# verlab/accelerated_features

Hardware: AMD Instinct MI355X
Metric: frames/sec detectAndCompute+match (VGA, top_k=4096) (higher is better)
Workload: dtype f32; 1 GPU; VGA 640x480 sparse top_k=4096, batch=64 per GPU: detectAndCompute + MNN match of the 32 consecutive frame pairs (BASELINE configs[1]); batch_per_gpu=64, height=480, width=640, top_k=4096, weights=synthetic (tests/fixtures.py), barrier=none (one rank), concurrent_lanes=True, lanes=2

## Files before the change

### accelerated_features_amd/csrc/k_match_f16.hip

```cpp
#include "../../include/xfeat_hip.h"
#include "kernels.hpp"
#include <type_traits>

namespace xfh {

void prof_begin(Profiler* p, int which, hipStream_t st);
void prof_end(Profiler* p, int which, hipStream_t st, double flops, double bytes);

typedef float f32x16 __attribute__((ext_vector_type(16)));
typedef _Float16 f16x8 __attribute__((ext_vector_type(8)));
typedef _Float16 f16x4 __attribute__((ext_vector_type(4)));


constexpr int FT_COLS = 256;
constexpr int FT_DS = 72;
constexpr float F16_C = 1.03f * 0.0009765625f;
constexpr float F16_KAPPA = 1.0e-5f;
constexpr float F16_UNIT_SCALE = 256.f;

__device__ inline int fpair_count(const int32_t* n, int idx, int cap) {
    if (!n) return cap;
    const int v = n[idx];
    return v < 0 ? 0 : (v > cap ? cap : v);
}
__device__ inline float f16_scale(float maxnorm) {
    if (!(maxnorm > 0.f)) return 1.f;
    int e;
    (void)frexpf(maxnorm, &e);
    return ldexpf(1.f, 8 - e);
}

template <bool CVT>
__global__ __launch_bounds__(256) void mnn_prep_kernel(const float* __restrict__ d1, size_t ps1, const float* __restrict__ d2, size_t ps2,
                                                       const int32_t* __restrict__ n1p, const int32_t* __restrict__ n2p, int n_stride, int n_off2,
                                                       int N1, int N2, _Float16* __restrict__ a16, _Float16* __restrict__ b16,
                                                       float* __restrict__ na, float* __restrict__ nb, unsigned* __restrict__ nmax ) {
    __shared__ float wmax[4];
    const int p = blockIdx.y, side = blockIdx.z, P = gridDim.y;
    const int N = side ? N2 : N1;
    const int n = side ? fpair_count(n2p, p * n_stride + n_off2, N2) : fpair_count(n1p, p * n_stride, N1);
    const int sub = threadIdx.x & 15;
    if (blockIdx.x * 256 >= n) return;
    const float* src = (side ? d2 + (size_t)p * ps2 : d1 + (size_t)p * ps1);
    const float sc = CVT ? f16_scale(__uint_as_float(nmax[side * P + p])) : 0.f;
    float m = 0.f;
#pragma unroll 4
    for (int it = 0; it < 16; ++it) {
        const int row = blockIdx.x * 256 + it * 16 + (threadIdx.x >> 4);
        float s = 0.f;
        if (row < n) {
            const float4 v = *reinterpret_cast<const float4*>(src + (size_t)row * 64 + sub * 4);
            if (CVT) {
                f16x4 o;
                o[0] = (_Float16)(v.x * sc); o[1] = (_Float16)(v.y * sc); o[2] = (_Float16)(v.z * sc); o[3] = (_Float16)(v.w * sc);
                *reinterpret_cast<f16x4*>((side ? b16 : a16) + ((size_t)p * N + row) * 64 + sub * 4) = o;
            } else {
                s = v.x * v.x + v.y * v.y + v.z * v.z + v.w * v.w;
            }
        }
        if (!CVT) {
            s += __shfl_xor(s, 8, 64);
            s += __shfl_xor(s, 4, 64);
            s += __shfl_xor(s, 2, 64);
            s += __shfl_xor(s, 1, 64);
            const float nrm = sqrtf(s) * 1.000001f;
            if (row < n && sub == 0) (side ? nb : na)[(size_t)p * N + row] = nrm;
            if (row < n) m = fmaxf(m, nrm);
        }
    }
    if (!CVT) {
        m = fmaxf(m, __shfl_xor(m, 16, 64));
        m = fmaxf(m, __shfl_xor(m, 32, 64));
        if ((threadIdx.x & 63) == 0) wmax[threadIdx.x >> 6] = m;
        __syncthreads();
        if (threadIdx.x == 0)
            atomicMax(&nmax[side * P + p], __float_as_uint(fmaxf(fmaxf(wmax[0], wmax[1]), fmaxf(wmax[2], wmax[3]))));
    }
}

constexpr float F16_STORE_SCALE = 0.25f;
__device__ inline _Float16 f16_up(float x) { return (_Float16)(__builtin_fmaf(__builtin_fabsf(x), 0.0009765625f, x) + 5.9604644775390625e-8f); }
__device__ inline _Float16 f16_down(float x) { return (_Float16)(__builtin_fmaf(__builtin_fabsf(x), -0.0009765625f, x) - 5.9604644775390625e-8f); }

__device__ inline float max16(const f32x16& v) {
    const float a = fmaxf(fmaxf(v[0], v[1]), v[2]);
    const float b = fmaxf(fmaxf(v[3], v[4]), v[5]);
    const float c = fmaxf(fmaxf(v[6], v[7]), v[8]);
    const float d = fmaxf(fmaxf(v[9], v[10]), v[11]);
    const float e = fmaxf(fmaxf(v[12], v[13]), v[14]);
    const float f = fmaxf(fmaxf(a, b), c);
    const float g = fmaxf(fmaxf(d, e), v[15]);
    return fmaxf(f, g);
}

__device__ inline float xhalf_max(float v) {
    const auto r = __builtin_amdgcn_permlane32_swap(__float_as_uint(v), __float_as_uint(v), false, false);
    return fmaxf(__uint_as_float(r[0]), __uint_as_float(r[1]));
}

struct PairWindow { float two_c, two_k; };
__device__ inline PairWindow pair_window(float unit_bound, const unsigned* __restrict__ nmax, int P, int p, bool row_side) {
    PairWindow w;
    if (unit_bound > 0.f) {
        const float ss = F16_UNIT_SCALE * F16_UNIT_SCALE;
        w.two_c = 2.f * F16_C * ss * unit_bound;
        w.two_k = 2.f * F16_KAPPA * ss * unit_bound * unit_bound;
    } else {
        const float ma = __uint_as_float(nmax[p]), mb = __uint_as_float(nmax[P + p]);
        const float ss = f16_scale(ma) * f16_scale(mb);
        w.two_c = 2.f * F16_C * ss * (row_side ? mb : ma);
        w.two_k = 2.f * F16_KAPPA * ss * ma * mb;
    }
    w.two_c = __uint_as_float(__builtin_amdgcn_readfirstlane(__float_as_uint(w.two_c)));
    w.two_k = __uint_as_float(__builtin_amdgcn_readfirstlane(__float_as_uint(w.two_k)));
    return w;
}

#define XFH_KEEP_FRAGS(f) asm volatile("" :: "v"(f[0]), "v"(f[1]), "v"(f[2]), "v"(f[3]))
#define XFH_WAVE_SYNC() __builtin_amdgcn_wave_barrier()

constexpr int FT_TILES = FT_COLS / 32;
__global__ __launch_bounds__(512) void mnn_f16_sweep_kernel(const _Float16* __restrict__ a16, size_t sa16, const _Float16* __restrict__ b16, size_t sb16,
                                                            const int32_t* __restrict__ n1p, const int32_t* __restrict__ n2p, int n_stride, int n_off2,
                                                            int N1, int N2, int ncc, int nsplit, int P,
                                                            unsigned* __restrict__ colmaxh, unsigned* __restrict__ rowmaxh,
                                                            _Float16* __restrict__ R, _Float16* __restrict__ C
#if XFH_CODE_SHIFT > 0
                                                            , int cold
#endif
                                                            ) {
#if XFH_CODE_SHIFT > 0
    kernel_entry_hooks(cold);
#endif
    __shared__ __attribute__((aligned(16))) _Float16 Dl[FT_COLS * FT_DS];
    __shared__ float colx[8][FT_COLS];
    __shared__ int next_block;
    const int tid = threadIdx.x, lane = tid & 63, half = lane >> 5, l31 = lane & 31;
    const int wave = __builtin_amdgcn_readfirstlane(tid >> 6);
    int p, item;
    if (!xcd_group_map(blockIdx.x, ncc * nsplit, P, p, item)) return;
    const int cc = item / nsplit, rs = item - cc * nsplit;
    const int n1 = fpair_count(n1p, p * n_stride, N1);
    const int n2 = fpair_count(n2p, p * n_stride + n_off2, N2);
    const int c0 = cc * FT_COLS;
    if (n1 <= 0 || n2 <= 0 || c0 >= n2) return;
    const _Float16* A = a16 + (size_t)p * sa16;
    const _Float16* Bm = b16 + (size_t)p * sb16;
    const int ncb32 = ceil_div(N2, 32), nrb32 = ceil_div(N1, 32);
    const int ntile = min(FT_TILES, ceil_div(n2 - c0, 32));
    const int bps = ceil_div(ceil_div(n1, 32), nsplit);
    const int blk_lo = rs * bps, nblock = min(ceil_div(n1, 32), blk_lo + bps);
    if (blk_lo >= nblock) return;
    if (tid == 0) next_block = blk_lo + 8;
    {
        uint4 v[4];
#pragma unroll
        for (int i = 0; i < 4; ++i) {
            const int e = tid + i * 512;
            v[i] = *reinterpret_cast<const uint4*>(Bm + (size_t)min(c0 + (e >> 3), n2 - 1) * 64 + (e & 7) * 8);
        }
#pragma unroll
        for (int i = 0; i < 4; ++i) {
            const int e = tid + i * 512;
            *reinterpret_cast<uint4*>(Dl + (e >> 3) * FT_DS + (e & 7) * 8) = v[i];
        }
#pragma unroll
        for (int i = 0; i < 4; ++i) (&colx[0][0])[tid + i * 512] = -INFINITY;
    }
    f16x8 a[4], an[4];
    int blk = blk_lo + wave, nxt;
    if (blk < nblock) {
        const int row = min(blk * 32 + l31, n1 - 1);
#pragma unroll
        for (int kk = 0; kk < 4; ++kk) an[kk] = *reinterpret_cast<const f16x8*>(A + (size_t)row * 64 + kk * 16 + half * 8);
    }
    __syncthreads();
    float* mycolx = &colx[wave][l31];
    const _Float16* bp0 = Dl + l31 * FT_DS + half * 8;
    while (blk < nblock) {
        {
            int t = 0;
            if (lane == 0) t = atomicAdd(&next_block, 1);
            nxt = __builtin_amdgcn_readfirstlane(t);
        }
#pragma unroll
        for (int kk = 0; kk < 4; ++kk) a[kk] = an[kk];
        if (nxt < nblock) {
            const int row = min(nxt * 32 + l31, n1 - 1);
#pragma unroll
            for (int kk = 0; kk < 4; ++kk) an[kk] = *reinterpret_cast<const f16x8*>(A + (size_t)row * 64 + kk * 16 + half * 8);
        }
        const int myrow = blk * 32 + l31;
        const __amdgpu_buffer_rsrc_t rC = __builtin_amdgcn_make_buffer_rsrc(C + ((size_t)p * nrb32 + blk) * N2 + c0, 0, (min(n2, c0 + FT_COLS) - c0) * 2, 0x00020000);
        const __amdgpu_buffer_rsrc_t rR = __builtin_amdgcn_make_buffer_rsrc(R + ((size_t)p * ncb32 + (c0 >> 5)) * N1, 0, FT_TILES * N1 * 2, 0x00020000);
        const int offC = half == 0 ? l31 * 2 : (int)0x80000000;
        const int offR = (half == 1 && myrow < n1) ? myrow * 2 : (int)0x80000000;
        float rowrun = -INFINITY;
        f16x8 bfrag[2][4];
#pragma unroll
        for (int kk = 0; kk < 4; ++kk) bfrag[0][kk] = *reinterpret_cast<const f16x8*>(bp0 + kk * 16);
        f32x16 acc, accT;
#define XFH_ROW_EPILOGUE(CT)                                                                              \
        {                                                                                                 \
            float rm = max16(accT);                                                                       \
            rm = fmaxf(rm, xhalf(rm));                                                                    \
            rowrun = fmaxf(rowrun, rm);                                                                   \
            __builtin_amdgcn_raw_buffer_store_b16(__builtin_bit_cast(short, f16_up(rm * F16_STORE_SCALE)), rR, offR, (CT) * N1 * 2, 0);       \
        }
#define XFH_INTERLEAVE_4x5()                                                                              \
        __builtin_amdgcn_sched_group_barrier(0x008, 1, 0); __builtin_amdgcn_sched_group_barrier(0x002, 5, 0);   \
        __builtin_amdgcn_sched_group_barrier(0x008, 1, 0); __builtin_amdgcn_sched_group_barrier(0x002, 5, 0);   \
        __builtin_amdgcn_sched_group_barrier(0x008, 1, 0); __builtin_amdgcn_sched_group_barrier(0x002, 5, 0);   \
        __builtin_amdgcn_sched_group_barrier(0x008, 1, 0); __builtin_amdgcn_sched_group_barrier(0x002, 5, 0);
#pragma unroll
        for (int ct = 0; ct < FT_TILES; ++ct) {
            if (ct < ntile) {
                if (ct + 1 < FT_TILES) {
#pragma unroll
                    for (int kk = 0; kk < 4; ++kk) bfrag[(ct + 1) & 1][kk] = *reinterpret_cast<const f16x8*>(bp0 + (ct + 1) * 32 * FT_DS + kk * 16);
                }
#pragma unroll
                for (int r = 0; r < 16; ++r) acc[r] = 0.f;
#pragma unroll
                for (int kk = 0; kk < 4; ++kk) acc = __builtin_amdgcn_mfma_f32_32x32x16_f16(a[kk], bfrag[ct & 1][kk], acc, 0, 0, 0);
                if (ct > 0) XFH_ROW_EPILOGUE(ct - 1)
                XFH_INTERLEAVE_4x5()
                __builtin_amdgcn_sched_barrier(0);
#pragma unroll
                for (int r = 0; r < 16; ++r) accT[r] = 0.f;
#pragma unroll
                for (int kk = 0; kk < 4; ++kk) accT = __builtin_amdgcn_mfma_f32_32x32x16_f16(bfrag[ct & 1][kk], a[kk], accT, 0, 0, 0);
                {
                    float cm = max16(acc);
                    cm = fmaxf(cm, xhalf(cm));
                    __hip_atomic_fetch_max(mycolx + ct * 32, cm, __ATOMIC_RELAXED, __HIP_MEMORY_SCOPE_WORKGROUP);
                    __builtin_amdgcn_raw_buffer_store_b16(__builtin_bit_cast(short, f16_up(cm * F16_STORE_SCALE)), rC, offC + ct * 64, 0, 0);
                }
                XFH_INTERLEAVE_4x5()
                __builtin_amdgcn_sched_barrier(0);
                XFH_KEEP_FRAGS(bfrag[ct & 1]);
            }
        }
        XFH_ROW_EPILOGUE(ntile - 1)
#undef XFH_ROW_EPILOGUE
#undef XFH_INTERLEAVE_4x5
        if (half == 0 && myrow < n1) atomicMax(&rowmaxh[(size_t)p * N1 + myrow], float_ord(rowrun));
        blk = nxt;
    }
    __syncthreads();
    if (tid < FT_COLS && c0 + tid < n2) {
        float k = colx[0][tid];
#pragma unroll
        for (int w = 1; w < 8; ++w) k = fmaxf(k, colx[w][tid]);
        atomicMax(&colmaxh[(size_t)p * N2 + c0 + tid], float_ord(k));
    }
}

constexpr int S2_T = 32;
constexpr int S2_GROUP = 32 * S2_T;
constexpr int S2_WAVES = 4;
constexpr int S2_TILES = 4;
constexpr int S2_COLS = 32 * S2_TILES;
constexpr int S2_XP = 33;
__host__ __device__ inline int s2_c_blocks(int N1) { return ceil_div(N1, S2_GROUP) * 32; }
__global__ __launch_bounds__(64 * S2_WAVES) __attribute__((amdgpu_waves_per_eu(2, 2)))
void mnn_f16_sweep2_kernel(const _Float16* __restrict__ a16, size_t sa16, const _Float16* __restrict__ b16, size_t sb16,
                           const int32_t* __restrict__ n1p, const int32_t* __restrict__ n2p, int n_stride, int n_off2,
                           int N1, int N2, int ncc, int ngq, int P,
                           unsigned* __restrict__ colmaxh, unsigned* __restrict__ rowmaxh, _Float16* __restrict__ R, _Float16* __restrict__ C) {
    __shared__ __attribute__((aligned(16))) _Float16 Dl2[S2_COLS * FT_DS];
    __shared__ __attribute__((aligned(16))) _Float16 af[S2_WAVES][64 * FT_DS];
    const int tid = threadIdx.x, lane = tid & 63, half = lane >> 5, l31 = lane & 31;
    const int wave = __builtin_amdgcn_readfirstlane(tid >> 6);
    int p, item;
    if (!xcd_group_map(blockIdx.x, ncc * ngq, P, p, item)) return;
    const int cc = item / ngq, gq = item - cc * ngq;
    const int n1 = fpair_count(n1p, p * n_stride, N1);
    const int n2 = fpair_count(n2p, p * n_stride + n_off2, N2);
    const int c0 = cc * S2_COLS;
    if (n1 <= 0 || n2 <= 0 || c0 >= n2 || gq * S2_WAVES * S2_GROUP >= n1) return;
    const _Float16* A = a16 + (size_t)p * sa16;
    const _Float16* Bm = b16 + (size_t)p * sb16;
    const int ncb32 = ceil_div(N2, 32);
    {
        constexpr int NP = S2_COLS * 8 / (64 * S2_WAVES);
        uint4 v[NP];
#pragma unroll
        for (int i = 0; i < NP; ++i) {
            const int e = tid + i * (64 * S2_WAVES);
            v[i] = *reinterpret_cast<const uint4*>(Bm + (size_t)min(c0 + (e >> 3), n2 - 1) * 64 + (e & 7) * 8);
        }
#pragma unroll
        for (int i = 0; i < NP; ++i) {
            const int e = tid + i * (64 * S2_WAVES);
            *reinterpret_cast<uint4*>(Dl2 + (e >> 3) * FT_DS + (e & 7) * 8) = v[i];
        }
    }
    const int g = gq * S2_WAVES + wave;
    const int blk_lo = g * S2_T, nblock = min(ceil_div(n1, 32), blk_lo + S2_T);
    f16x8 ax[4], ay[4], anx[4], any_[4];
#define XFH_S2_REQUEST(BLK)                                                                                \
    {                                                                                                     \
         \
        _Pragma("unroll") for (int q = 0; q < 4; ++q) {                                                   \
            const int e = q * 64 + lane, rx = min((BLK) * 32 + (e >> 3), n1 - 1), ry = (BLK) + 1 < nblock ? min((BLK) * 32 + 32 + (e >> 3), n1 - 1) : rx;       \
            anx[q] = *reinterpret_cast<const f16x8*>(A + (size_t)rx * 64 + (e & 7) * 8);                  \
            any_[q] = *reinterpret_cast<const f16x8*>(A + (size_t)ry * 64 + (e & 7) * 8);                 \
        }                                                                                                 \
    }
    XFH_S2_REQUEST(min(blk_lo, max(nblock - 1, 0)))
    __syncthreads();
    if (blk_lo >= nblock) return;
    const _Float16* bp0 = Dl2 + l31 * FT_DS + half * 8;
    _Float16* afw = af[wave];
    f32x16 M[S2_TILES];
#pragma unroll
    for (int ct = 0; ct < S2_TILES; ++ct)
#pragma unroll
        for (int r = 0; r < 16; ++r) M[ct][r] = -INFINITY;
    const __amdgpu_buffer_rsrc_t rR = __builtin_amdgcn_make_buffer_rsrc(R + ((size_t)p * ncb32 + (c0 >> 5)) * N1, 0, min(S2_TILES, ncb32 - (c0 >> 5)) * N1 * 2, 0x00020000);
    constexpr int NSTEP = 4 * S2_TILES;
    f16x8 bq[4];
    bq[0] = *reinterpret_cast<const f16x8*>(bp0);
    bq[1] = *reinterpret_cast<const f16x8*>(bp0 + 16);
    for (int blk = blk_lo; blk < nblock; blk += 2) {
#pragma unroll
        for (int q = 0; q < 4; ++q) {
            const int e = q * 64 + lane;
            *reinterpret_cast<f16x8*>(afw + (e >> 3) * FT_DS + (e & 7) * 8) = anx[q];
            *reinterpret_cast<f16x8*>(afw + (32 + (e >> 3)) * FT_DS + (e & 7) * 8) = any_[q];
        }
        XFH_WAVE_SYNC();
#pragma unroll
        for (int kk = 0; kk < 4; ++kk) {
            ax[kk] = *reinterpret_cast<const f16x8*>(afw + l31 * FT_DS + kk * 16 + half * 8);
            ay[kk] = *reinterpret_cast<const f16x8*>(afw + (32 + l31) * FT_DS + kk * 16 + half * 8);
        }
        XFH_WAVE_SYNC();
        XFH_S2_REQUEST(min(blk + 2, nblock - 1))
        const int myrow = blk * 32 + lane;
        const int offR = myrow < n1 ? myrow * 2 : (int)0x80000000;
        const int arow = half && blk + 1 >= nblock ? min(blk * 32 + l31, n1 - 1) : min(myrow, n1 - 1);
        float rowrun = -INFINITY;
        f32x16 accx[2], accy[2];
#define XFH_S2_FENCE() __builtin_amdgcn_sched_barrier(0)
#define XFH_S2_M(CT, R0, R1) { _Pragma("unroll") for (int r = (R0); r < (R1); ++r) M[CT][r] = fmaxf(fmaxf(M[CT][r], accx[(CT) & 1][r]), accy[(CT) & 1][r]); }
#define XFH_S2_PIN2(CT, R0) asm volatile("" : "+v"(M[CT][R0]), "+v"(M[CT][(R0) + 1]))
#define XFH_S2_PIN10(CT, R0) asm volatile("" : "+v"(M[CT][R0]), "+v"(M[CT][(R0) + 1]), "+v"(M[CT][(R0) + 2]), "+v"(M[CT][(R0) + 3]), "+v"(M[CT][(R0) + 4]), "+v"(M[CT][(R0) + 5]), \
                                                "+v"(M[CT][(R0) + 6]), "+v"(M[CT][(R0) + 7]), "+v"(M[CT][(R0) + 8]), "+v"(M[CT][(R0) + 9]))
#define XFH_S2_EPI0(CT) rx_ = max16(accx[(CT) & 1]); XFH_S2_M(CT, 0, 2) XFH_S2_PIN2(CT, 0); asm volatile("" : "+v"(rx_));
#define XFH_S2_EPI1(CT) ry_ = max16(accy[(CT) & 1]); XFH_S2_M(CT, 2, 4) XFH_S2_PIN2(CT, 2); asm volatile("" : "+v"(ry_));
#define XFH_S2_EPI2(CT)                                                                                   \
            {                                                                                             \
                const auto sw_ = __builtin_amdgcn_permlane32_swap(__float_as_uint(rx_), __float_as_uint(ry_), false, false);       \
                const float rm_ = fmaxf(__uint_as_float(sw_[0]), __uint_as_float(sw_[1]));                \
                rowrun = fmaxf(rowrun, rm_);                                                              \
                __builtin_amdgcn_raw_buffer_store_b16(__builtin_bit_cast(short, f16_up(rm_ * F16_STORE_SCALE)), rR, offR + (CT) * N1 * 2, 0, 0);    \
            }                                                                                             \
            XFH_S2_M(CT, 4, 6) XFH_S2_PIN2(CT, 4); asm volatile("" : "+v"(rowrun));
#define XFH_S2_EPI3(CT) XFH_S2_M(CT, 6, 16) XFH_S2_PIN10(CT, 6);
        float rx_ = 0.f, ry_ = 0.f;
#pragma unroll
        for (int ct = 0; ct < S2_TILES; ++ct)
#pragma unroll
        for (int kk = 0; kk < 4; ++kk) {
            const int s_ = 4 * ct + kk;
            {
                const int sn = (s_ + 2) % NSTEP;
                bq[(s_ + 2) & 3] = *reinterpret_cast<const f16x8*>(bp0 + (sn >> 2) * 32 * FT_DS + (sn & 3) * 16);
            }
            f32x16& cx = accx[ct & 1];
            f32x16& cy = accy[ct & 1];
            if (kk == 0) {
#pragma unroll
                for (int r = 0; r < 16; ++r) { cx[r] = 0.f; cy[r] = 0.f; }
            }
            cx = __builtin_amdgcn_mfma_f32_32x32x16_f16(bq[s_ & 3], ax[kk], cx, 0, 0, 0);
            cy = __builtin_amdgcn_mfma_f32_32x32x16_f16(bq[s_ & 3], ay[kk], cy, 0, 0, 0);
            asm volatile("" : "+v"(cx), "+v"(cy));
            XFH_S2_FENCE();
            if (ct > 0) {
                if (kk == 0) { XFH_S2_EPI0(ct - 1) }
                if (kk == 1) { XFH_S2_EPI1(ct - 1) }
                if (kk == 2) { XFH_S2_EPI2(ct - 1) }
                if (kk == 3) { XFH_S2_EPI3(ct - 1) }
                XFH_S2_FENCE();
            }
            asm volatile("" :: "v"(bq[s_ & 3]));
        }
        {
            XFH_S2_EPI0(S2_TILES - 1)
            XFH_S2_EPI1(S2_TILES - 1)
            XFH_S2_EPI2(S2_TILES - 1)
            XFH_S2_EPI3(S2_TILES - 1)
        }
        XFH_S2_FENCE();
        XFH_KEEP_FRAGS(ax);
        XFH_KEEP_FRAGS(ay);
#undef XFH_S2_FENCE
#undef XFH_S2_PIN2
#undef XFH_S2_PIN10
#undef XFH_S2_M
#undef XFH_S2_EPI0
#undef XFH_S2_EPI1
#undef XFH_S2_EPI2
#undef XFH_S2_EPI3
        atomicMax(&rowmaxh[(size_t)p * N1 + arow], float_ord(rowrun));
    }
    float* xw = reinterpret_cast<float*>(af[wave]);
    static_assert(32 * S2_XP * 4 <= 64 * FT_DS * 2, "the flush tile lives in the wave's fragment rows");
    const bool vec_ok = (N2 & 7) == 0;
    _Float16* crow = C + ((size_t)p * s2_c_blocks(N1) + g * 32 + l31) * N2 + c0;
#pragma unroll
    for (int ct = 0; ct < S2_TILES; ++ct) {
#pragma unroll
        for (int r = 0; r < 16; ++r) xw[l31 * S2_XP + (r & 3) + 8 * (r >> 2) + 4 * half] = M[ct][r];
        XFH_WAVE_SYNC();
        float cm = xw[(16 * half) * S2_XP + l31];
#pragma unroll
        for (int t = 1; t < 16; ++t) cm = fmaxf(cm, xw[(16 * half + t) * S2_XP + l31]);
        cm = fmaxf(cm, xhalf(cm));
        const int col = c0 + ct * 32 + l31;
        if (half == 0 && col < n2) atomicMax(&colmaxh[(size_t)p * N2 + col], float_ord(cm));
        const int cs = ct * 32 + 16 * half;
        _Float16 o[16];
#pragma unroll
        for (int t = 0; t < 16; ++t) o[t] = f16_up(xw[l31 * S2_XP + 16 * half + t] * F16_STORE_SCALE);
#pragma unroll
        for (int q = 0; q < 2; ++q) {
            f16x8 v;
#pragma unroll
            for (int t = 0; t < 8; ++t) v[t] = o[8 * q + t];
            if (vec_ok && c0 + cs + 8 * q + 8 <= n2) *reinterpret_cast<f16x8*>(crow + cs + 8 * q) = v;
            else {
#pragma unroll
                for (int t = 0; t < 8; ++t)
                    if (c0 + cs + 8 * q + t < n2) crow[cs + 8 * q + t] = v[t];
            }
        }
        XFH_WAVE_SYNC();
    }
}

__global__ __launch_bounds__(256) void mnn_f16_thr_kernel(float unit_bound, const int32_t* __restrict__ n1p, const int32_t* __restrict__ n2p, int n_stride, int n_off2,
                                                          int N1, int N2, int P, const float* __restrict__ na, const float* __restrict__ nb,
                                                          const unsigned* __restrict__ nmax, const unsigned* __restrict__ rowmaxh, const unsigned* __restrict__ colmaxh,
                                                          _Float16* __restrict__ thr_row, _Float16* __restrict__ thr_col) {
    const int p = blockIdx.y, side = blockIdx.z, i = blockIdx.x * 256 + threadIdx.x;
    const int N = side ? N2 : N1;
    if (i >= (side ? fpair_count(n2p, p * n_stride + n_off2, N2) : fpair_count(n1p, p * n_stride, N1))) return;
    const PairWindow w = pair_window(unit_bound, nmax, P, p, side == 0);
    const float nx = unit_bound > 0.f ? unit_bound : (side ? nb : na)[(size_t)p * N + i];
    (side ? thr_col : thr_row)[(size_t)p * N + i] = f16_down((ord_float((side ? colmaxh : rowmaxh)[(size_t)p * N + i]) - fmaf(w.two_c, nx, w.two_k)) * F16_STORE_SCALE);
}

constexpr int RF_ROUND = 512;
constexpr int RF_CHUNK = 4096;
constexpr int RF_QUEUE = 1024;
constexpr int RF_XS = 68;
constexpr int RF_WAVES = 2;
__global__ __launch_bounds__(64 * RF_WAVES) __attribute__((amdgpu_waves_per_eu(4, 8))) void mnn_f16_refine_kernel(
    const float* __restrict__ d1, size_t ps1, const float* __restrict__ d2, size_t ps2, const int32_t* __restrict__ n1p,
    const int32_t* __restrict__ n2p, int n_stride, int n_off2, int N1, int N2, int nyb_max, int c_strided, int P,
    const _Float16* __restrict__ thr_row, const _Float16* __restrict__ thr_col, const _Float16* __restrict__ R,
    const _Float16* __restrict__ C, unsigned long long* __restrict__ rowkey, unsigned long long* __restrict__ colkey) {
    __shared__ unsigned short queue[RF_WAVES][RF_QUEUE];
    __shared__ __attribute__((aligned(16))) float tile[RF_WAVES][32 * RF_XS];
    const int lane = threadIdx.x & 63, half = lane >> 5, l31 = lane & 31;
    const int wv = __builtin_amdgcn_readfirstlane(threadIdx.x >> 6);
    int p, item;
    if (!xcd_group_map(blockIdx.x, 2 * (nyb_max / RF_WAVES), P, p, item)) return;
    const int side = item / (nyb_max / RF_WAVES), yb = (item - side * (nyb_max / RF_WAVES)) * RF_WAVES + wv;
    const int n1 = fpair_count(n1p, p * n_stride, N1);
    const int n2 = fpair_count(n2p, p * n_stride + n_off2, N2);
    if (n1 <= 0 || n2 <= 0) return;
    const int nX = side ? n2 : n1, nY = side ? n1 : n2, NX = side ? N2 : N1;
    const bool strided = side && c_strided;
    const int ybase = strided ? (yb >> 5) * S2_GROUP + (yb & 31) : yb * 32, ystep = strided ? 32 : 1;
    if (ybase >= nY) return;
    const float* X = side ? d2 + (size_t)p * ps2 : d1 + (size_t)p * ps1;
    const float* Y = side ? d1 + (size_t)p * ps1 : d2 + (size_t)p * ps2;
    const _Float16* M = (side ? C + (size_t)p * (c_strided ? s2_c_blocks(N1) : ceil_div(N1, 32)) * N2 : R + (size_t)p * ceil_div(N2, 32) * N1) + (size_t)yb * NX;
    const _Float16* T = side ? thr_col + (size_t)p * N2 : thr_row + (size_t)p * N1;
    unsigned long long* key = side ? colkey + (size_t)p * N2 : rowkey + (size_t)p * N1;
    const bool vec_ok = (NX & 7) == 0;
    unsigned short* q = queue[wv];
    float* xt = tile[wv];
    const __amdgpu_buffer_rsrc_t rM = __builtin_amdgcn_make_buffer_rsrc(const_cast<_Float16*>(M), 0, nX * 2, 0x00020000);
    const __amdgpu_buffer_rsrc_t rT = __builtin_amdgcn_make_buffer_rsrc(const_cast<_Float16*>(T), 0, nX * 2, 0x00020000);
    const __amdgpu_buffer_rsrc_t rX = __builtin_amdgcn_make_buffer_rsrc(const_cast<float*>(X), 0, nX * 256, 0x00020000);
    const __amdgpu_buffer_rsrc_t rY = __builtin_amdgcn_make_buffer_rsrc(const_cast<float*>(Y), 0, nY * 256, 0x00020000);

    const int trow = lane >> 4, tq = lane & 15;
    auto rows_to_operand = [&](const __amdgpu_buffer_rsrc_t& rs, auto row_of, float (&reg)[32]) {
        uint4 v[8];
#pragma unroll
        for (int i = 0; i < 8; ++i) v[i] = __builtin_bit_cast(uint4, __builtin_amdgcn_raw_buffer_load_b128(rs, row_of(4 * i + trow) * 256 + tq * 16, 0, 0));
#pragma unroll
        for (int i = 0; i < 8; ++i) *reinterpret_cast<uint4*>(xt + (4 * i + trow) * RF_XS + tq * 4) = v[i];
#pragma unroll
        for (int t = 0; t < 8; ++t) {
            const float4 f = *reinterpret_cast<const float4*>(xt + l31 * RF_XS + half * 32 + t * 4);
            reg[4 * t] = f.x; reg[4 * t + 1] = f.y; reg[4 * t + 2] = f.z; reg[4 * t + 3] = f.w;
        }
    };
    float yreg[32];
    rows_to_operand(rY, [&](int r) { return ybase + r * ystep; }, yreg);
    const bool ragged = ybase + 31 * ystep >= nY;

    for (int xc = 0; xc < nX; xc += RF_CHUNK) {
        int cnt = 0;
        auto drain = [&]() {
            for (int e0 = 0; e0 < cnt; e0 += 32) {
                float xreg[32];
                rows_to_operand(rX, [&](int r) { return xc + (int)q[min(e0 + r, cnt - 1)]; }, xreg);
                f32x16 acc;
#pragma unroll
                for (int r = 0; r < 16; ++r) acc[r] = 0.f;
#pragma unroll
                for (int s_ = 0; s_ < 32; ++s_) acc = __builtin_amdgcn_mfma_f32_32x32x2f32(yreg[s_], xreg[s_], acc, 0, 0, 0);
                if (ragged) {
#pragma unroll
                    for (int r = 0; r < 16; ++r)
                        if (ybase + ((r & 3) + 8 * (r >> 2) + 4 * half) * ystep >= nY) acc[r] = -INFINITY;
                }
                const float m = max16(acc);
                int ry = 0;
#pragma unroll
                for (int r = 15; r >= 0; --r)
                    if (acc[r] == m) ry = (r & 3) + 8 * (r >> 2);
                unsigned long long k = ((unsigned long long)float_ord(m) << 32) | (0xffffffffu - (unsigned)(ybase + (ry + 4 * half) * ystep));
                k = u64_max(k, xhalf_u64(k));
                const int e = e0 + l31;
                if (half == 0 && e < cnt) atomicMax(&key[xc + q[e]], k);
            }
            cnt = 0;
        };
        const int nround = ceil_div(min(RF_CHUNK, nX - xc), RF_ROUND);
        auto issue = [&](auto vec, int r, f16x8& m, f16x8& t) {
            const int xb = xc + r * RF_ROUND + lane * 8;
            if constexpr (decltype(vec)::value) {
                m = __builtin_bit_cast(f16x8, __builtin_amdgcn_raw_buffer_load_b128(rM, xb * 2, 0, 0));
                t = __builtin_bit_cast(f16x8, __builtin_amdgcn_raw_buffer_load_b128(rT, xb * 2, 0, 0));
            } else {
#pragma unroll
                for (int j = 0; j < 8; ++j) {
                    m[j] = __builtin_bit_cast(_Float16, __builtin_amdgcn_raw_buffer_load_b16(rM, (xb + j) * 2, 0, 0));
                    t[j] = __builtin_bit_cast(_Float16, __builtin_amdgcn_raw_buffer_load_b16(rT, (xb + j) * 2, 0, 0));
                }
            }
        };
        auto test = [&](int r, const f16x8& m, const f16x8& t) {
            if (cnt > RF_QUEUE - RF_ROUND) drain();
            const int xl = r * RF_ROUND + lane * 8;
            const int left = nX - (xc + xl);
            const f16x8 d = m - t;
            const uint4 db = __builtin_bit_cast(uint4, d);
            const unsigned dw[4] = {db.x, db.y, db.z, db.w};
#pragma unroll
            for (int j = 0; j < 8; ++j) {
                const bool neg = (dw[j >> 1] >> (15 + 16 * (j & 1))) & 1u;
                const unsigned long long bal = __ballot(!neg && j < left);
                if (bal) {
                    if ((bal >> lane) & 1ull) q[cnt + __popcll(bal & ((1ull << lane) - 1ull))] = (unsigned short)(xl + j);
                    cnt += __popcll(bal);
                }
            }
        };
        auto scan = [&](auto vec) {
            constexpr int NB = decltype(vec)::value ? 4 : 1;
            for (int r0 = 0; r0 < nround; r0 += NB) {
                f16x8 m4[NB], t4[NB];
#pragma unroll
                for (int k = 0; k < NB; ++k) issue(vec, r0 + k, m4[k], t4[k]);
#pragma unroll
                for (int k = 0; k < NB; ++k)
                    if (r0 + k < nround) test(r0 + k, m4[k], t4[k]);
            }
        };
        if (vec_ok) scan(std::true_type{});
        else scan(std::false_type{});
        drain();
    }
}

void launch_match_f16(const MatchWs& ws, const float* d1, size_t ps1, const float* d2, size_t ps2, const uint16_t* d1_16, const uint16_t* d2_16,
                      const int32_t* n1, const int32_t* n2, int n_stride, int n_off2, int P, int N1, int N2, hipStream_t st, Profiler* prof, int sweep_form) {
    const bool prepared = d1_16 && d2_16;
    const _Float16* a16 = prepared ? reinterpret_cast<const _Float16*>(d1_16) : ws.a16;
    const _Float16* b16 = prepared ? reinterpret_cast<const _Float16*>(d2_16) : ws.b16;
    const size_t sa = prepared ? ps1 : (size_t)N1 * 64, sb = prepared ? ps2 : (size_t)N2 * 64;
    const float ub = prepared ? 1.00001f : 0.f;
    if (!prepared) {
        prof_begin(prof, XFH_SPAN_MATCH_PREP, st);
        const dim3 g(ceil_div(N1 > N2 ? N1 : N2, 256), P, 2);
        mnn_prep_kernel<false><<<g, 256, 0, st>>>(d1, ps1, d2, ps2, n1, n2, n_stride, n_off2, N1, N2, ws.a16, ws.b16, ws.na, ws.nb, ws.nmax);
        mnn_prep_kernel<true><<<g, 256, 0, st>>>(d1, ps1, d2, ps2, n1, n2, n_stride, n_off2, N1, N2, ws.a16, ws.b16, ws.na, ws.nb, ws.nmax);
        prof_end(prof, XFH_SPAN_MATCH_PREP, st, 0, 0);
    }
    prof_begin(prof, XFH_SPAN_MATCH_SWEEP, st);
    const int ngroup = ceil_div(N1, S2_GROUP), ncc2 = ceil_div(N2, S2_COLS);
    const bool one = sweep_form == 2 || ((long)P * ncc2 * ngroup >= 8L * num_cus() && sweep_form != 1);
    if (one) {
        const int ngq = ceil_div(ngroup, S2_WAVES);
        mnn_f16_sweep2_kernel<<<xcd_grid_size(ncc2 * ngq, P), 64 * S2_WAVES, 0, st>>>(a16, sa, b16, sb, n1, n2, n_stride, n_off2, N1, N2, ncc2, ngq, P,
                                                                                    ws.colmaxh, ws.rowmaxh, reinterpret_cast<_Float16*>(ws.R), reinterpret_cast<_Float16*>(ws.C));
    } else {
    const int ncc = ceil_div(N2, FT_COLS);
    const int nsplit = max(1, min(ceil_div(2 * num_cus(), ncc * P), ceil_div(N1, 256)));
    mnn_f16_sweep_kernel<<<xcd_grid_size(ncc * nsplit, P), 512, 0, st>>>(a16, sa, b16, sb, n1, n2, n_stride, n_off2, N1, N2, ncc, nsplit, P,
                                                                        ws.colmaxh, ws.rowmaxh, reinterpret_cast<_Float16*>(ws.R), reinterpret_cast<_Float16*>(ws.C)
#if XFH_CODE_SHIFT > 0
                                                                        , g_debug_cold
#endif
                                                                        );
    }
    prof_end(prof, XFH_SPAN_MATCH_SWEEP, st, 0, 0);
    const int nyb = ceil_div(max(ceil_div(N2, 32), one ? s2_c_blocks(N1) : ceil_div(N1, 32)), RF_WAVES) * RF_WAVES;
    prof_begin(prof, XFH_SPAN_MATCH_REFINE, st);
    mnn_f16_thr_kernel<<<dim3(ceil_div(N1 > N2 ? N1 : N2, 256), P, 2), 256, 0, st>>>(ub, n1, n2, n_stride, n_off2, N1, N2, P, ws.na, ws.nb, ws.nmax, ws.rowmaxh, ws.colmaxh,
                                                                                        reinterpret_cast<_Float16*>(ws.thr_row), reinterpret_cast<_Float16*>(ws.thr_col));
    mnn_f16_refine_kernel<<<xcd_grid_size(2 * (nyb / RF_WAVES), P), 64 * RF_WAVES, 0, st>>>(d1, ps1, d2, ps2, n1, n2, n_stride, n_off2, N1, N2, nyb, one ? 1 : 0, P,
                                                                          reinterpret_cast<const _Float16*>(ws.thr_row), reinterpret_cast<const _Float16*>(ws.thr_col), reinterpret_cast<const _Float16*>(ws.R),
                                                                          reinterpret_cast<const _Float16*>(ws.C), ws.rowkey, ws.colkey);
    prof_end(prof, XFH_SPAN_MATCH_REFINE, st, 0, 0);
}

}
```

Before: 57610 frames/s.

## Software-pipeline MNN refine kernel: prefetch scan windows and X rows, split Y operand

Restructures the f16 MNN refine kernel. The Y rows and the first window of mask/threshold loads are now issued before the pair counts are read, so the initial memory latency overlaps the early-exit checks. A rolling 8-round window replaces the fixed 4096 chunk, with the next window prefetched while candidates are queued. During drain the next 32 X rows are loaded while the current MFMA block runs, and the Y operand is split into two 16-element halves to cut register use. The vector/scalar path is now a template parameter chosen on the host from N1|N2. This adds complexity, a smaller queue (768), and loads that are issued even for blocks that will exit early.

```diff
diff --git a/accelerated_features_amd/csrc/k_match_f16.hip b/accelerated_features_amd/csrc/k_match_f16.hip
--- a/accelerated_features_amd/csrc/k_match_f16.hip
+++ b/accelerated_features_amd/csrc/k_match_f16.hip
@@ -455,132 +455,155 @@
 }
 
 constexpr int RF_ROUND = 512;
-constexpr int RF_CHUNK = 4096;
-constexpr int RF_QUEUE = 1024;
+constexpr int RF_WINDOW = 8;
+constexpr int RF_QUEUE = 768;
 constexpr int RF_XS = 68;
 constexpr int RF_WAVES = 2;
+
+template <bool VEC>
 __global__ __launch_bounds__(64 * RF_WAVES) __attribute__((amdgpu_waves_per_eu(4, 8))) void mnn_f16_refine_kernel(
     const float* __restrict__ d1, size_t ps1, const float* __restrict__ d2, size_t ps2, const int32_t* __restrict__ n1p,
     const int32_t* __restrict__ n2p, int n_stride, int n_off2, int N1, int N2, int nyb_max, int c_strided, int P,
     const _Float16* __restrict__ thr_row, const _Float16* __restrict__ thr_col, const _Float16* __restrict__ R,
     const _Float16* __restrict__ C, unsigned long long* __restrict__ rowkey, unsigned long long* __restrict__ colkey) {
-    __shared__ unsigned short queue[RF_WAVES][RF_QUEUE];
+    constexpr int NB = VEC ? RF_WINDOW : 1;
+    __shared__ __attribute__((aligned(16))) unsigned short queue[RF_WAVES][RF_QUEUE];
     __shared__ __attribute__((aligned(16))) float tile[RF_WAVES][32 * RF_XS];
     const int lane = threadIdx.x & 63, half = lane >> 5, l31 = lane & 31;
     const int wv = __builtin_amdgcn_readfirstlane(threadIdx.x >> 6);
     int p, item;
     if (!xcd_group_map(blockIdx.x, 2 * (nyb_max / RF_WAVES), P, p, item)) return;
     const int side = item / (nyb_max / RF_WAVES), yb = (item - side * (nyb_max / RF_WAVES)) * RF_WAVES + wv;
+    const int NX = side ? N2 : N1, NY = side ? N1 : N2;
+    const bool strided = side && c_strided;
+    const int ybase = strided ? (yb >> 5) * S2_GROUP + (yb & 31) : yb * 32, ystep = strided ? 32 : 1;
+    const int nblk = side ? (c_strided ? s2_c_blocks(N1) : ceil_div(N1, 32)) : ceil_div(N2, 32);
+    const bool has_blk = yb < nblk;
+    const float* X = side ? d2 + (size_t)p * ps2 : d1 + (size_t)p * ps1;
+    const float* Y = side ? d1 + (size_t)p * ps1 : d2 + (size_t)p * ps2;
+    const _Float16* M = (side ? C : R) + ((size_t)p * nblk + (has_blk ? yb : 0)) * NX;
+    const _Float16* T = side ? thr_col + (size_t)p * N2 : thr_row + (size_t)p * N1;
+    unsigned long long* key = side ? colkey + (size_t)p * N2 : rowkey + (size_t)p * N1;
+    unsigned short* q = queue[wv];
+    float* xt = tile[wv];
+    const __amdgpu_buffer_rsrc_t rM = __builtin_amdgcn_make_buffer_rsrc(const_cast<_Float16*>(M), 0, has_blk ? NX * 2 : 0, 0x00020000);
+    const __amdgpu_buffer_rsrc_t rT = __builtin_amdgcn_make_buffer_rsrc(const_cast<_Float16*>(T), 0, NX * 2, 0x00020000);
+    const __amdgpu_buffer_rsrc_t rX = __builtin_amdgcn_make_buffer_rsrc(const_cast<float*>(X), 0, NX * 256, 0x00020000);
+    const __amdgpu_buffer_rsrc_t rY = __builtin_amdgcn_make_buffer_rsrc(const_cast<float*>(Y), 0, NY * 256, 0x00020000);
+
+    const int trow = lane >> 4, tq = lane & 15;
+    auto load_rows = [&](const __amdgpu_buffer_rsrc_t& rs, auto row_of, uint4 (&v)[8]) {
+#pragma unroll
+        for (int i = 0; i < 8; ++i) v[i] = __builtin_bit_cast(uint4, __builtin_amdgcn_raw_buffer_load_b128(rs, row_of(4 * i + trow) * 256 + tq * 16, 0, 0));
+    };
+    auto tile_write = [&](const uint4 (&v)[8]) {
+#pragma unroll
+        for (int i = 0; i < 8; ++i) *reinterpret_cast<uint4*>(xt + (4 * i + trow) * RF_XS + tq * 4) = v[i];
+    };
+    auto tile_read = [&](int hq, float (&reg)[16]) {
+#pragma unroll
+        for (int t = 0; t < 4; ++t) {
+            const float4 f = *reinterpret_cast<const float4*>(xt + l31 * RF_XS + half * 32 + hq * 16 + t * 4);
+            reg[4 * t] = f.x; reg[4 * t + 1] = f.y; reg[4 * t + 2] = f.z; reg[4 * t + 3] = f.w;
+        }
+    };
+    f16x8 mw[NB], tw[NB];
+    auto issue = [&](int xw) {
+#pragma unroll
+        for (int k = 0; k < NB; ++k) {
+            const int xb = xw + k * RF_ROUND + lane * 8;
+            if constexpr (VEC) {
+                mw[k] = __builtin_bit_cast(f16x8, __builtin_amdgcn_raw_buffer_load_b128(rM, xb * 2, 0, 0));
+                tw[k] = __builtin_bit_cast(f16x8, __builtin_amdgcn_raw_buffer_load_b128(rT, xb * 2, 0, 0));
+            } else {
+#pragma unroll
+                for (int j = 0; j < 8; ++j) {
+                    mw[k][j] = __builtin_bit_cast(_Float16, __builtin_amdgcn_raw_buffer_load_b16(rM, (xb + j) * 2, 0, 0));
+                    tw[k][j] = __builtin_bit_cast(_Float16, __builtin_amdgcn_raw_buffer_load_b16(rT, (xb + j) * 2, 0, 0));
+                }
+            }
+        }
+    };
+    uint4 yraw[8];
+    load_rows(rY, [&](int r) { return ybase + r * ystep; }, yraw);
+    issue(0);
+
     const int n1 = fpair_count(n1p, p * n_stride, N1);
     const int n2 = fpair_count(n2p, p * n_stride + n_off2, N2);
-    if (n1 <= 0 || n2 <= 0) return;
-    const int nX = side ? n2 : n1, nY = side ? n1 : n2, NX = side ? N2 : N1;
-    const bool strided = side && c_strided;
-    const int ybase = strided ? (yb >> 5) * S2_GROUP + (yb & 31) : yb * 32, ystep = strided ? 32 : 1;
-    if (ybase >= nY) return;
-    const float* X = side ? d2 + (size_t)p * ps2 : d1 + (size_t)p * ps1;
-    const float* Y = side ? d1 + (size_t)p * ps1 : d2 + (size_t)p * ps2;
-    const _Float16* M = (side ? C + (size_t)p * (c_strided ? s2_c_blocks(N1) : ceil_div(N1, 32)) * N2 : R + (size_t)p * ceil_div(N2, 32) * N1) + (size_t)yb * NX;
-    const _Float16* T = side ? thr_col + (size_t)p * N2 : thr_row + (size_t)p * N1;
-    unsigned long long* key = side ? colkey + (size_t)p * N2 : rowkey + (size_t)p * N1;
-    const bool vec_ok = (NX & 7) == 0;
-    unsigned short* q = queue[wv];
-    float* xt = tile[wv];
-    const __amdgpu_buffer_rsrc_t rM = __builtin_amdgcn_make_buffer_rsrc(const_cast<_Float16*>(M), 0, nX * 2, 0x00020000);
-    const __amdgpu_buffer_rsrc_t rT = __builtin_amdgcn_make_buffer_rsrc(const_cast<_Float16*>(T), 0, nX * 2, 0x00020000);
-    const __amdgpu_buffer_rsrc_t rX = __builtin_amdgcn_make_buffer_rsrc(const_cast<float*>(X), 0, nX * 256, 0x00020000);
-    const __amdgpu_buffer_rsrc_t rY = __builtin_amdgcn_make_buffer_rsrc(const_cast<float*>(Y), 0, nY * 256, 0x00020000);
-
-    const int trow = lane >> 4, tq = lane & 15;
-    auto rows_to_operand = [&](const __amdgpu_buffer_rsrc_t& rs, auto row_of, float (&reg)[32]) {
-        uint4 v[8];
-#pragma unroll
-        for (int i = 0; i < 8; ++i) v[i] = __builtin_bit_cast(uint4, __builtin_amdgcn_raw_buffer_load_b128(rs, row_of(4 * i + trow) * 256 + tq * 16, 0, 0));
-#pragma unroll
-        for (int i = 0; i < 8; ++i) *reinterpret_cast<uint4*>(xt + (4 * i + trow) * RF_XS + tq * 4) = v[i];
-#pragma unroll
-        for (int t = 0; t < 8; ++t) {
-            const float4 f = *reinterpret_cast<const float4*>(xt + l31 * RF_XS + half * 32 + t * 4);
-            reg[4 * t] = f.x; reg[4 * t + 1] = f.y; reg[4 * t + 2] = f.z; reg[4 * t + 3] = f.w;
-        }
-    };
-    float yreg[32];
-    rows_to_operand(rY, [&](int r) { return ybase + r * ystep; }, yreg);
-    const bool ragged = ybase + 31 * ystep >= nY;
-
-    for (int xc = 0; xc < nX; xc += RF_CHUNK) {
-        int cnt = 0;
-        auto drain = [&]() {
-            for (int e0 = 0; e0 < cnt; e0 += 32) {
-                float xreg[32];
-                rows_to_operand(rX, [&](int r) { return xc + (int)q[min(e0 + r, cnt - 1)]; }, xreg);
-                f32x16 acc;
-#pragma unroll
-                for (int r = 0; r < 16; ++r) acc[r] = 0.f;
-#pragma unroll
-                for (int s_ = 0; s_ < 32; ++s_) acc = __builtin_amdgcn_mfma_f32_32x32x2f32(yreg[s_], xreg[s_], acc, 0, 0, 0);
-                if (ragged) {
-#pragma unroll
-                    for (int r = 0; r < 16; ++r)
-                        if (ybase + ((r & 3) + 8 * (r >> 2) + 4 * half) * ystep >= nY) acc[r] = -INFINITY;
+    const int nX = side ? n2 : n1, nY = side ? n1 : n2;
+    if (n1 > 0 && n2 > 0 && ybase < nY) {
+        float yreg[2][16];
+        tile_write(yraw);
+        tile_read(0, yreg[0]);
+        tile_read(1, yreg[1]);
+        const bool ragged = ybase + 31 * ystep >= nY;
+        int cnt = 0, xq = 0;
+        for (int xw = 0;;) {
+            int stop = NB;
+#pragma unroll
+            for (int k = 0; k < NB; ++k) {
+                const int xl = xw - xq + k * RF_ROUND + lane * 8;
+                const int left = nX - (xq + xl);
+                if (k < stop && xw + k * RF_ROUND < nX) {
+                    if (cnt > RF_QUEUE - RF_ROUND) stop = k;
+                    else {
+                        const f16x8 d = mw[k] - tw[k];
+                        const uint4 db = __builtin_bit_cast(uint4, d);
+                        const unsigned dw[4] = {db.x, db.y, db.z, db.w};
+#pragma unroll
+                        for (int j = 0; j < 8; ++j) {
+                            const bool neg = (dw[j >> 1] >> (15 + 16 * (j & 1))) & 1u;
+                            const unsigned long long bal = __ballot(!neg && j < left);
+                            if (bal) {
+                                if ((bal >> lane) & 1ull) q[cnt + __popcll(bal & ((1ull << lane) - 1ull))] = (unsigned short)(xl + j);
+                                cnt += __popcll(bal);
+                            }
+                        }
+                    }
                 }
-                const float m = max16(acc);
-                int ry = 0;
-#pragma unroll
-                for (int r = 15; r >= 0; --r)
-                    if (acc[r] == m) ry = (r & 3) + 8 * (r >> 2);
-                unsigned long long k = ((unsigned long long)float_ord(m) << 32) | (0xffffffffu - (unsigned)(ybase + (ry + 4 * half) * ystep));
-                k = u64_max(k, xhalf_u64(k));
-                const int e = e0 + l31;
-                if (half == 0 && e < cnt) atomicMax(&key[xc + q[e]], k);
-            }
-            cnt = 0;
-        };
-        const int nround = ceil_div(min(RF_CHUNK, nX - xc), RF_ROUND);
-        auto issue = [&](auto vec, int r, f16x8& m, f16x8& t) {
-            const int xb = xc + r * RF_ROUND + lane * 8;
-            if constexpr (decltype(vec)::value) {
-                m = __builtin_bit_cast(f16x8, __builtin_amdgcn_raw_buffer_load_b128(rM, xb * 2, 0, 0));
-                t = __builtin_bit_cast(f16x8, __builtin_amdgcn_raw_buffer_load_b128(rT, xb * 2, 0, 0));
-            } else {
-#pragma unroll
-                for (int j = 0; j < 8; ++j) {
-                    m[j] = __builtin_bit_cast(_Float16, __builtin_amdgcn_raw_buffer_load_b16(rM, (xb + j) * 2, 0, 0));
-                    t[j] = __builtin_bit_cast(_Float16, __builtin_amdgcn_raw_buffer_load_b16(rT, (xb + j) * 2, 0, 0));
+            }
+            const int xn = xw + (stop < NB ? stop : NB) * RF_ROUND;
+            const bool done = xn >= nX;
+            if (done || cnt > RF_QUEUE - RF_ROUND || xn + NB * RF_ROUND - xq > 65536) {
+              if (cnt > 0) {
+                uint4 xraw[8];
+                load_rows(rX, [&](int r) { return xq + (int)q[min(r, cnt - 1)]; }, xraw);
+                for (int e0 = 0; e0 < cnt; e0 += 32) {
+                    tile_write(xraw);
+                    load_rows(rX, [&](int r) { return xq + (int)q[min(e0 + 32 + r, cnt - 1)]; }, xraw);
+                    f32x16 acc;
+#pragma unroll
+                    for (int r = 0; r < 16; ++r) acc[r] = 0.f;
+#pragma unroll
+                    for (int hq = 0; hq < 2; ++hq) {
+                        float xreg[16];
+                        tile_read(hq, xreg);
+#pragma unroll
+                        for (int s_ = 0; s_ < 16; ++s_) acc = __builtin_amdgcn_mfma_f32_32x32x2f32(yreg[hq][s_], xreg[s_], acc, 0, 0, 0);
+                    }
+                    if (ragged) {
+#pragma unroll
+                        for (int r = 0; r < 16; ++r)
+                            if (ybase + ((r & 3) + 8 * (r >> 2) + 4 * half) * ystep >= nY) acc[r] = -INFINITY;
+                    }
+                    const float m = max16(acc);
+                    int ry = 0;
+#pragma unroll
+                    for (int r = 15; r >= 0; --r)
+                        if (acc[r] == m) ry = (r & 3) + 8 * (r >> 2);
+                    unsigned long long k = ((unsigned long long)float_ord(m) << 32) | (0xffffffffu - (unsigned)(ybase + (ry + 4 * half) * ystep));
+                    k = u64_max(k, xhalf_u64(k));
+                    const int e = e0 + l31;
+                    if (half == 0 && e < cnt) atomicMax(&key[xq + q[min(e, cnt - 1)]], k);
                 }
-            }
-        };
-        auto test = [&](int r, const f16x8& m, const f16x8& t) {
-            if (cnt > RF_QUEUE - RF_ROUND) drain();
-            const int xl = r * RF_ROUND + lane * 8;
-            const int left = nX - (xc + xl);
-            const f16x8 d = m - t;
-            const uint4 db = __builtin_bit_cast(uint4, d);
-            const unsigned dw[4] = {db.x, db.y, db.z, db.w};
-#pragma unroll
-            for (int j = 0; j < 8; ++j) {
-                const bool neg = (dw[j >> 1] >> (15 + 16 * (j & 1))) & 1u;
-                const unsigned long long bal = __ballot(!neg && j < left);
-                if (bal) {
-                    if ((bal >> lane) & 1ull) q[cnt + __popcll(bal & ((1ull << lane) - 1ull))] = (unsigned short)(xl + j);
-                    cnt += __popcll(bal);
-                }
-            }
-        };
-        auto scan = [&](auto vec) {
-            constexpr int NB = decltype(vec)::value ? 4 : 1;
-            for (int r0 = 0; r0 < nround; r0 += NB) {
-                f16x8 m4[NB], t4[NB];
-#pragma unroll
-                for (int k = 0; k < NB; ++k) issue(vec, r0 + k, m4[k], t4[k]);
-#pragma unroll
-                for (int k = 0; k < NB; ++k)
-                    if (r0 + k < nround) test(r0 + k, m4[k], t4[k]);
-            }
-        };
-        if (vec_ok) scan(std::true_type{});
-        else scan(std::false_type{});
-        drain();
+              }
+              cnt = 0;
+              xq = xn;
+            }
+            if (done) break;
+            xw = xn;
+            issue(xw);
+        }
     }
 }
 
@@ -620,7 +643,8 @@
     prof_begin(prof, XFH_SPAN_MATCH_REFINE, st);
     mnn_f16_thr_kernel<<<dim3(ceil_div(N1 > N2 ? N1 : N2, 256), P, 2), 256, 0, st>>>(ub, n1, n2, n_stride, n_off2, N1, N2, P, ws.na, ws.nb, ws.nmax, ws.rowmaxh, ws.colmaxh,
                                                                                         reinterpret_cast<_Float16*>(ws.thr_row), reinterpret_cast<_Float16*>(ws.thr_col));
-    mnn_f16_refine_kernel<<<xcd_grid_size(2 * (nyb / RF_WAVES), P), 64 * RF_WAVES, 0, st>>>(d1, ps1, d2, ps2, n1, n2, n_stride, n_off2, N1, N2, nyb, one ? 1 : 0, P,
+    const auto kern = ((N1 | N2) & 7) == 0 ? mnn_f16_refine_kernel<true> : mnn_f16_refine_kernel<false>;
+    kern<<<xcd_grid_size(2 * (nyb / RF_WAVES), P), 64 * RF_WAVES, 0, st>>>(d1, ps1, d2, ps2, n1, n2, n_stride, n_off2, N1, N2, nyb, one ? 1 : 0, P,
                                                                           reinterpret_cast<const _Float16*>(ws.thr_row), reinterpret_cast<const _Float16*>(ws.thr_col), reinterpret_cast<const _Float16*>(ws.R),
                                                                           reinterpret_cast<const _Float16*>(ws.C), ws.rowkey, ws.colkey);
     prof_end(prof, XFH_SPAN_MATCH_REFINE, st, 0, 0);
```

Measured after the change: 57670 frames/s (median of 2 runs). No clear change (+0.1%).
